# akanimax/thr3ed_atom

Measured on AMD Instinct MI355X. Metric: ray-samples/sec (fwd+bwd) training step, 800x800 images @ 128^3 SH-2 ReLU field, higher is better.
Workload: dtype f32

## Files before the change

### thr3ed_atom_amd/csrc/relu_field_kernels.hip

```cpp
#include <hip/hip_runtime.h>
#include <stdint.h>

#include <atomic>
#include <climits>
#include <cmath>
#include <cstdlib>
#include <type_traits>

#include "relu_field.h"

namespace {

#ifndef RF_FWD_WAVES
#define RF_FWD_WAVES 4
#endif
#ifndef RF_EMIT_WAVES
#define RF_EMIT_WAVES 6
#endif
#ifndef RF_EMIT_G
#define RF_EMIT_G 2
#endif
constexpr int kWave = 64;
constexpr int kWavesPerBlock = 4;
constexpr int kBlock = kWave * kWavesPerBlock;
// ... 2019 lines not shown
}

template <int K, bool ADAM, bool ONE_ROUND, int TH = kBrickThreads, int BX = 8, bool MIRROR = false>
__device__ __forceinline__ void brick_flush(const GridArgs& g, const BrickArgs& a, const float* acc, bool any, int X0, int Y0, int Z0,
                                            float* gdens, float* gfeat) {
  static_assert(!MIRROR || (ADAM && ONE_ROUND && BX == 4), "the mirror write-out rides on the one-round optimizer flush of 4 x 8 x 8 bricks");
  constexpr int C = 3 * K + 1;
  constexpr int CS = (C + 3) / 4 * 4;
  const int B = ONE_ROUND ? 8 : (1 << a.shift);
  const int SY = brick_row_stride(B, C), SX = brick_slab_stride(B, C);
  const int tid = threadIdx.x;
  const bool split = g.layout == RF_LAYOUT_SPLIT;
  if (split && (C & 3) == 0 && (g.dstride & 3) == 0 && (C == 4 || (g.fstride & 3) == 0)) {
    constexpr int QN = C / 4;
    constexpr int QR = QN > 1 ? QN - 1 : 1;
    const int nq = (BX == 4 ? 4 : B) * B * B * QN;
    auto quad_of = [&](int i, int& fx, int& fy, int& fz, int& qd) -> bool {
      const int col = (i >> a.shift) / QN, r = i - col * (B * QN);
      const bool first = r < B;
      fz = first ? r : (r - B) / QR;
      qd = first ? 0 : 1 + (r - B) - fz * QR;
      fx = col >> a.shift;
      fy = col & (B - 1);
      return i < nq && X0 + fx < g.X && Y0 + fy < g.Y && Z0 + fz < g.Z;
    };
    if constexpr (ADAM) {
      constexpr int U = (QN == 7) ? 4 : 1;
      const AdamArgs& ad = a.adam;
      if constexpr (ONE_ROUND) {
        unsigned int bo[QN];
        int lds_at[QN];
        float4 p4[QN];
        vf4 m4[QN], v4[QN];
#pragma unroll
        for (int u = 0; u < QN; ++u) {
          int fx, fy, fz, qd;
          if (u == 0) {
            fx = tid >> 6;
            fy = (tid >> 3) & 7;
            fz = tid & 7;
            qd = 0;
          } else {
            const int j = (u - 1) * TH + tid, col = j / 48, r = j - col * 48;
            fz = r / 6;
            qd = 1 + r - 6 * fz;
            fx = col >> 3;
            fy = col & 7;
          }
          const bool ok = X0 + fx < g.X && Y0 + fy < g.Y && Z0 + fz < g.Z;
          const unsigned int lin = ok ? node_lin(g, X0 + fx, Y0 + fy, Z0 + fz) : 0u;
          const unsigned int o = u == 0 ? __umul24(lin, (unsigned)g.dstride) : __umul24(lin, (unsigned)g.fstride) + 4u * (unsigned)(qd - 1);
          bo[u] = ok ? o * 4u : 0xffffffffu;
          lds_at[u] = fx * SX + fy * SY + fz * CS + 4 * qd;
        }
#pragma unroll
        for (int u = 0; u < QN; ++u) {
          if (bo[u] != 0xffffffffu) {
            const char* pb = reinterpret_cast<const char*>(u == 0 ? ad.p1 : ad.p2);
            const char* mb = reinterpret_cast<const char*>(u == 0 ? ad.m1 : ad.m2);
            const char* vb = reinterpret_cast<const char*>(u == 0 ? ad.v1 : ad.v2);
            p4[u] = *reinterpret_cast<const float4*>(pb + bo[u]);
            m4[u] = __builtin_nontemporal_load(reinterpret_cast<const vf4*>(mb + bo[u]));
            v4[u] = __builtin_nontemporal_load(reinterpret_cast<const vf4*>(vb + bo[u]));
          }
        }
#pragma unroll
        for (int u = 0; u < QN; ++u) {
          if (bo[u] == 0xffffffffu) continue;
          const float4 gq = any ? *reinterpret_cast<const float4*>(&acc[lds_at[u]]) : make_float4(0.f, 0.f, 0.f, 0.f);
          float gg[4] = {gq.x, gq.y, gq.z, gq.w};
          float pn[4] = {p4[u].x, p4[u].y, p4[u].z, p4[u].w};
          if (u == 0 && g.mode == RF_DENSITY_ABS) {
            const float dv = pn[0] * g.rho;
            gg[0] = (dv > 0.f) ? gg[0] : ((dv < 0.f) ? -gg[0] : 0.0f);
          }
          vf4 mn, vn;
#pragma unroll
          for (int c = 0; c < 4; ++c) {
            float mm = m4[u][c], vv = v4[u][c];
            adam_update(pn[c], mm, vv, gg[c], ad.step, ad.b1, ad.b2, ad.eps, ad.inv_bc2_sqrt);
            mn[c] = mm;
            vn[c] = vv;
          }
          char* pb = reinterpret_cast<char*>(u == 0 ? ad.p1 : ad.p2);
          char* mb = reinterpret_cast<char*>(u == 0 ? ad.m1 : ad.m2);
          char* vb = reinterpret_cast<char*>(u == 0 ? ad.v1 : ad.v2);
          *reinterpret_cast<float4*>(pb + bo[u]) = make_float4(pn[0], pn[1], pn[2], pn[3]);
          __builtin_nontemporal_store(mn, reinterpret_cast<vf4*>(mb + bo[u]));
          __builtin_nontemporal_store(vn, reinterpret_cast<vf4*>(vb + bo[u]));
          if constexpr (MIRROR) *reinterpret_cast<float4*>(const_cast<float*>(&acc[lds_at[u]])) = make_float4(pn[0], pn[1], pn[2], pn[3]);
        }
        if constexpr (MIRROR) {
          __syncthreads();
          constexpr int F = 3 * K, FQ = 2 * F, CQ = FQ + 2;
          for (int i = tid; i < 32 * CQ; i += TH) {
            const int col = i / CQ, r = i - col * CQ;
            const int fx = col >> 3, fy = col & 7;
            const float* img = acc + fx * SX + fy * SY;
            const unsigned int lin0 = node_lin(g, X0 + fx, Y0 + fy, Z0);
            float v[4];
            if (r < FQ) {
#pragma unroll
              for (int t = 0; t < 4; ++t) {
                const int e = 4 * r + t;
                const int nz = e / F, f = e - nz * F;
                const int colour = f / K, k = f - colour * K;
                v[t] = img[nz * CS + (k == 0 ? 1 + colour : 4 + colour * (K - 1) + (k - 1))];
              }
              *reinterpret_cast<float4*>(gfeat + (size_t)(__umul24(lin0, (unsigned)F) + 4u * (unsigned)r)) = make_float4(v[0], v[1], v[2], v[3]);
            } else {
              const int z0 = 4 * (r - FQ);
#pragma unroll
              for (int t = 0; t < 4; ++t) v[t] = img[(z0 + t) * CS];
              *reinterpret_cast<float4*>(gdens + (size_t)(lin0 + (unsigned)z0)) = make_float4(v[0], v[1], v[2], v[3]);
            }
          }
        }
        return;
      } else {
      for (int i0 = tid; i0 < nq; i0 += TH * U) {
        unsigned int off[U];
        float4 p4[U];
        vf4 m4[U], v4[U];
#pragma unroll
        for (int u = 0; u < U; ++u) {
          int fx, fy, fz, qd;
          const bool ok = quad_of(i0 + u * TH, fx, fy, fz, qd);
          const unsigned int lin = ok ? node_lin(g, X0 + fx, Y0 + fy, Z0 + fz) : 0u;
          const unsigned int o = qd == 0 ? lin * (unsigned)g.dstride : (lin * (unsigned)g.fstride + 4u * (unsigned)(qd - 1)) | 0x80000000u;
          off[u] = ok ? o : 0xffffffffu;
        }
#pragma unroll
        for (int u = 0; u < U; ++u) {
          if (off[u] != 0xffffffffu) {
            const bool rest = off[u] >> 31;
            const unsigned int o = off[u] & 0x7fffffffu;
#ifdef RF_BRICK_PROFILE
            if (a.stagger & 0x10000) { p4[u] = make_float4(0.f, 0.f, 0.f, 0.f); m4[u] = vf4{0.f, 0.f, 0.f, 0.f}; v4[u] = vf4{1.f, 1.f, 1.f, 1.f}; continue; }
#endif
            p4[u] = *reinterpret_cast<const float4*>((rest ? ad.p2 : ad.p1) + o);
            m4[u] = __builtin_nontemporal_load(reinterpret_cast<const vf4*>((rest ? ad.m2 : ad.m1) + o));
            v4[u] = __builtin_nontemporal_load(reinterpret_cast<const vf4*>((rest ? ad.v2 : ad.v1) + o));
          }
        }
#pragma unroll
        for (int u = 0; u < U; ++u) {
          if (off[u] == 0xffffffffu) continue;
          const bool rest = off[u] >> 31;
          const unsigned int o = off[u] & 0x7fffffffu;
          int fx, fy, fz, qd;
          quad_of(i0 + u * TH, fx, fy, fz, qd);
          const float4 gq = any ? *reinterpret_cast<const float4*>(&acc[fx * SX + fy * SY + fz * CS + 4 * qd]) : make_float4(0.f, 0.f, 0.f, 0.f);
          float gg[4] = {gq.x, gq.y, gq.z, gq.w};
          float pn[4] = {p4[u].x, p4[u].y, p4[u].z, p4[u].w};
          if (!rest && g.mode == RF_DENSITY_ABS) {
            const float dv = pn[0] * g.rho;
            gg[0] = (dv > 0.f) ? gg[0] : ((dv < 0.f) ? -gg[0] : 0.0f);
          }
          vf4 mn, vn;
#ifdef RF_BRICK_PROFILE
          if (a.stagger & 0x40000) {
#pragma unroll
            for (int c = 0; c < 4; ++c) { mn[c] = m4[u][c] + gg[c]; vn[c] = v4[u][c]; pn[c] += gg[c]; }
          } else
#endif
#pragma unroll
          for (int c = 0; c < 4; ++c) {
            float mm = m4[u][c], vv = v4[u][c];
            adam_update(pn[c], mm, vv, gg[c], ad.step, ad.b1, ad.b2, ad.eps, ad.inv_bc2_sqrt);
            mn[c] = mm;
            vn[c] = vv;
          }
#ifdef RF_BRICK_PROFILE
          if (a.stagger & 0x20000) { if (pn[0] == 123.456f) *reinterpret_cast<float4*>((rest ? ad.p2 : ad.p1) + o) = make_float4(mn[0], vn[1], pn[2], pn[3]); continue; }
#endif
          *reinterpret_cast<float4*>((rest ? ad.p2 : ad.p1) + o) = make_float4(pn[0], pn[1], pn[2], pn[3]);
          __builtin_nontemporal_store(mn, reinterpret_cast<vf4*>((rest ? ad.m2 : ad.m1) + o));
          __builtin_nontemporal_store(vn, reinterpret_cast<vf4*>((rest ? ad.v2 : ad.v1) + o));
        }
      }
      }
      return;
    }
    for (int i = tid; i < nq; i += TH) {
      int fx, fy, fz, qd;
      if (!quad_of(i, fx, fy, fz, qd)) continue;
      const long long lin = node_lin(g, X0 + fx, Y0 + fy, Z0 + fz);
      float4 v = any ? *reinterpret_cast<const float4*>(&acc[fx * SX + fy * SY + fz * CS + 4 * qd]) : make_float4(0.f, 0.f, 0.f, 0.f);
      if (qd == 0 && g.mode == RF_DENSITY_ABS) {
        const float dv = g.dens[lin * g.dstride] * g.rho;
        v.x = (dv > 0.f) ? v.x : ((dv < 0.f) ? -v.x : 0.0f);
      }
      const long long off = (qd == 0) ? lin * g.dstride : lin * g.fstride + 4 * (qd - 1);
      if (qd == 0) {
        float4* dst = reinterpret_cast<float4*>(gdens + off);
        if (a.accumulate) {
          const float4 o = *dst;
          v = make_float4(o.x + v.x, o.y + v.y, o.z + v.z, o.w + v.w);
        }
        *dst = v;
      } else {
        float4* dst = reinterpret_cast<float4*>(gfeat + off);
        if (a.accumulate) {
          const float4 o = *dst;
          v = make_float4(o.x + v.x, o.y + v.y, o.z + v.z, o.w + v.w);
        }
        const vf4 v4 = {v.x, v.y, v.z, v.w};
        __builtin_nontemporal_store(v4, reinterpret_cast<vf4*>(dst));
      }
    }
    return;
  }
  const int n_first = split ? 4 : 1;
  const int n_second = C - n_first;
  for (int pass = 0; pass < 2; ++pass) {
    const int nch = pass == 0 ? n_first : n_second;
    if (nch == 0) continue;
    const int run = B * nch;
    float* out = pass == 0 ? gdens : gfeat;
    const long long ostride = pass == 0 ? g.dstride : g.fstride;
    for (int i = tid; i < (BX == 4 ? 4 : B) * B * run; i += TH) {
      const int col = i / run, r = i - col * run;
      const int fz = r / nch, c2 = r - fz * nch;
      const int fx = col >> a.shift, fy = col & (B - 1);
      const int X = X0 + fx, Y = Y0 + fy, Z = Z0 + fz;
      if (X >= g.X || Y >= g.Y || Z >= g.Z) continue;
      int lds_c;
      if (split) {
        lds_c = pass * 4 + c2;
      } else if (pass == 0) {
        lds_c = 0;
      } else {
        const int col3 = c2 / K, kk = c2 - col3 * K;
        lds_c = (kk == 0) ? 1 + col3 : 4 + col3 * (K - 1) + (kk - 1);
      }
      const long long lin = node_lin(g, X, Y, Z);
      float v = any ? acc[fx * SX + fy * SY + fz * CS + lds_c] : 0.0f;
      if (lds_c == 0 && g.mode == RF_DENSITY_ABS) {
        const float dv = g.dens[lin * g.dstride] * g.rho;
        v = (dv > 0.f) ? v : ((dv < 0.f) ? -v : 0.0f);
      }
      float* dst = out + lin * ostride + (long long)c2 * (pass == 1 && !split ? a.fmul : 1);
      *dst = a.accumulate ? (*dst + v) : v;
    }
  }
}

__device__ __forceinline__ uint32_t lds_offset(const void* p) { return (uint32_t)(uintptr_t)p; }
template <int OFF>
__device__ __forceinline__ void lds_request_f32(float& v, uint32_t addr) {
  asm volatile("ds_read_b32 %0, %1 offset:%2" : "+v"(v) : "v"(addr), "n"(OFF));
}
__device__ __forceinline__ void lds_request_u8(uint32_t& v, uint32_t addr) {
  asm volatile("ds_read_u8 %0, %1" : "+v"(v) : "v"(addr));
}
__device__ __forceinline__ void lds_wait(uint32_t& a, uint32_t& b) { asm volatile("s_waitcnt lgkmcnt(0)" : "+v"(a), "+v"(b)); }
__device__ __forceinline__ void lds_wait(float& a, float& b, float& c, float& d, uint32_t& f) {
  asm volatile("s_waitcnt lgkmcnt(0)" : "+v"(a), "+v"(b), "+v"(c), "+v"(d), "+v"(f));
}
__device__ __forceinline__ void lds_wait(float& a, float& b, float& c, float& d, float& e, uint32_t& f) {
  asm volatile("s_waitcnt lgkmcnt(0)" : "+v"(a), "+v"(b), "+v"(c), "+v"(d), "+v"(e), "+v"(f));
}
__device__ __forceinline__ void lds_wait(float& a, float& b, float& c, float& d, float& e, float& e2, float& e3, uint32_t& f) {
  asm volatile("s_waitcnt lgkmcnt(0)" : "+v"(a), "+v"(b), "+v"(c), "+v"(d), "+v"(e), "+v"(e2), "+v"(e3), "+v"(f));
}

constexpr int kGatherBatch = 256;
constexpr int kGatherWtab = 24;
__host__ __device__ constexpr int gather_record_words(int C4) { return C4 + 8; }
typedef float f32x4 __attribute__((ext_vector_type(4)));

__host__ __device__ inline int gather_lds_words(int B, int C, int BX = 8) {
  const int C4 = (C + 3) / 4 * 4;
  const int gb = BX == 4 ? kGatherBatch / 2 : kGatherBatch;
  const int batch = gb * gather_record_words(C4) + (gb + 4) * kGatherWtab;
  const int image = BX == 4 ? 4 * brick_slab_stride(B, C) + 64 : brick_acc_words(B, C);
  return batch > image ? batch : image;
}

template <int K, bool ADAM, bool ONE_ROUND = false, bool SPLIT = false, int BX = 8, bool MIRROR = false>
__global__ __launch_bounds__(BX == 4 ? kBrickThreads / 2 : kBrickThreads, (K > 9 ? 2 : 4)) void brick_gather_kernel(GridArgs g, BrickArgs a, float* gdens, float* gfeat) {
  static_assert(BX == 8 || (BX == 4 && ONE_ROUND && !SPLIT), "4 x 8 x 8 bricks: 8-node y and z edges, one workgroup per brick");
  constexpr int TH = BX == 4 ? kBrickThreads / 2 : kBrickThreads;
  constexpr int NWV = TH / 64;
  constexpr int GB = TH / 2;
  constexpr int GROW = GB + 4;
  constexpr int C = 3 * K + 1;
  constexpr int C4 = (C + 3) / 4 * 4;
  constexpr int QW = record_quads(K);
  constexpr int QN = record_quads(1);
  constexpr int NT = (C4 + 15) / 16;
  static_assert(NT == 1 || NT == 2 || NT == 4, "one, two or four 16-channel blocks (SH degree 0 / base lists, 1-2, 3)");
  constexpr int CS = C4;
  constexpr int NW = GB / 64;
  constexpr bool SEP = BX == 4 && K == 9 && ONE_ROUND && !SPLIT;
  extern __shared__ __attribute__((aligned(16))) float acc[];
  float* rows = acc;
  float* wtab = acc + GB * gather_record_words(C4);
  __shared__ uint32_t s_tmask[GB];
  __shared__ unsigned char s_list[4 * NWV][GB + 24];
  __shared__ __attribute__((aligned(16))) int s_wstart[kMaxRangesKind], s_wcum[kMaxRangesKind + 8];
  __shared__ __attribute__((aligned(16))) int s_nstart[kMaxRangesKind], s_ncum[kMaxRangesKind + 8];
  __shared__ int s_part[4];
  const int B = ONE_ROUND ? 8 : (1 << a.shift);
  const int bshift = ONE_ROUND ? 3 : a.shift;
  const int SY = brick_row_stride(B, C), SX = brick_slab_stride(B, C);

  RF_PROF_START();
  const int tid = threadIdx.x;
  const int lane = tid & (kWave - 1);
  const int wave = tid >> 6;
  const int parts = SPLIT ? a.parts : 1;
  const int part = SPLIT ? (int)(blockIdx.x % (unsigned)parts) : 0;
  const int brick_local = SPLIT ? (int)(blockIdx.x / (unsigned)parts) : (int)blockIdx.x;
  const int brick = a.brick_first + brick_local;
  auto lists_of = [&](int nl) { return SPLIT ? (nl > part ? (nl - part + parts - 1) / parts : 0) : nl; };
  auto list_index = [&](int ll) { return SPLIT ? part + ll * parts : ll; };
  const int nwide_p = lists_of(a.nwide), nnarrow_p = lists_of(a.nnarrow);
  const int bz = brick % a.nbz, by = (brick / a.nbz) % a.nby, bx = brick / (a.nbz * a.nby);
  const int X0 = bx << (BX == 4 ? 2 : bshift), Y0 = by << bshift, Z0 = bz << bshift;
  {
    const int kind = tid >> 7, i = tid & 127;
    int start = 0, cnt = 0;
    if (tid < 256) {
      const int nl = kind ? nnarrow_p : nwide_p;
      if (i < kRangeEntries * nl) {
        const int l = nl == 1 ? 0 : i / kRangeEntries;
        const int li = list_index(l);
        const long long* offs = (!SPLIT && nl == 1) ? (kind ? a.narrow[0].offsets : a.wide[0].offsets) : (kind ? a.narrow[li].offsets : a.wide[li].offsets);
        brick_range_entry(a, offs, bx, by, bz, i - l * kRangeEntries, start, cnt);
      }
    }
    int cum = cnt;
#pragma unroll
    for (int d = 1; d < kWave; d <<= 1) {
      const int up = __shfl_up(cum, d);
      if (lane >= d) cum += up;
    }
    if (wave < 4 && lane == kWave - 1) s_part[wave] = cum;
    __syncthreads();
    if (tid < 256) {
      if (wave & 1) cum += s_part[wave - 1];
      int* st_ = kind ? s_nstart : s_wstart;
      int* cu_ = kind ? s_ncum : s_wcum;
      if (i < kMaxRangesKind) {
        st_[i] = start;
        cu_[i + 1] = cum;
      }
      if (i == 0) cu_[0] = 0;
    }
    __syncthreads();
  }
  const int total = s_wcum[kMaxRangesKind];
  const int total_d = s_ncum[kMaxRangesKind];
  bool any = total > 0 || total_d > 0;
  if (!SPLIT && !any && a.accumulate) return;
  RF_PROF_MARK(0);

  const int npz = B >> 2, npy = B >> 1;
  const int ntiles = BX == 4 ? 16 : (B * B * B) >> 4;
  const int mi = lane & 15;
  const int mdx = mi >> 3, mdy = (mi >> 2) & 1, mdz = mi & 3;
  const int kk = lane >> 4;
  const int jj = lane & 15;

  f32x4 accr[4][NT];
#pragma unroll
  for (int tl = 0; tl < 4; ++tl)
#pragma unroll
    for (int nt = 0; nt < NT; ++nt) accr[tl][nt] = f32x4{0.f, 0.f, 0.f, 0.f};
  f32x4 naccr = f32x4{0.f, 0.f, 0.f, 0.f};

  if (any) {
    const int nba = (total + GB - 1) / GB, nbd = (total_d + GB - 1) / GB;
    uint32_t wprev = 0x00ffffffu;
    const int rec_id = tid & (GB - 1);
    const int half = tid >= GB;

    auto stage = [&](auto expand_tag, auto blocks_tag, float4 q0, float4 q1, float4 q2, int nrec) {
      constexpr bool EXPAND = decltype(expand_tag)::value;
      constexpr bool BLOCKS = decltype(blocks_tag)::value;
      constexpr int RW = gather_record_words(EXPAND ? C4 : 4);
      if (half == 0) {
        uint32_t tm = 0, wnow = 0x00ffffffu;
        float* wcol = wtab + rec_id;
#pragma unroll
        for (int ax = 0; ax < 3; ++ax) {
          const int c1 = (int)((wprev >> (8 * ax)) & 0xffu);
          if (c1 != 0xff) {
            if (c1 >= 1) wcol[(ax * 8 + c1 - 1) * GROW] = 0.0f;
            if (c1 < (BX == 4 && ax == 0 ? 4 : B)) wcol[(ax * 8 + c1) * GROW] = 0.0f;
          }
        }
        if (rec_id < nrec) {
          const float idx[3] = {q0.x, q0.y, q0.z};
          const int org[3] = {X0, Y0, Z0};
          uint32_t pb[3];
          wnow = 0;
#pragma unroll
          for (int ax = 0; ax < 3; ++ax) {
            const float fl = floorf(idx[ax]);
            const int c = (int)fl - org[ax];
            const int sh = (BLOCKS && ax > 0) || ax == 2 ? 2 : 1;
            uint32_t bits = 0;
            if (c >= 0) {
              wcol[(ax * 8 + c) * GROW] = (fl + 1.0f) - idx[ax];
              bits |= 1u << (c >> sh);
            }
            if (c + 1 < (BX == 4 && ax == 0 ? 4 : B)) {
              wcol[(ax * 8 + c + 1) * GROW] = idx[ax] - fl;
              bits |= 1u << ((c + 1) >> sh);
            }
            pb[ax] = bits;
            wnow |= (uint32_t)(c + 1) << (8 * ax);
          }
          if constexpr (BLOCKS) {
            if (pb[0]) tm = ((pb[1] & 1u) ? pb[2] : 0u) | ((pb[1] & 2u) ? pb[2] << 2 : 0u);
          } else {
            uint32_t yz = 0;
#pragma unroll
            for (int py = 0; py < 4; ++py)
              if ((pb[1] >> py) & 1u) yz |= pb[2] << (py * npz);
#pragma unroll
            for (int px = 0; px < 4; ++px)
              if ((pb[0] >> px) & 1u) tm |= yz << (px * npy * npz);
          }
        }
        wprev = wnow;
        s_tmask[rec_id] = tm;
      }
      float* row = rows + rec_id * RW;
      if constexpr (EXPAND) {
        const float graw[3] = {q1.x, q1.y, q1.z};
        constexpr int NQ = C4 / 4;
        if (half == 0) {
          *reinterpret_cast<float4*>(row) = make_float4(q0.w, graw[0] * kC0, graw[1] * kC0, graw[2] * kC0);
        } else {
          float Y[16];
          sh_basis<K>(q1.w, q2.x, q2.y, Y);
#pragma unroll
          for (int q = 1; q < NQ; ++q) {
            float v[4];
#pragma unroll
            for (int x = 0; x < 4; ++x) v[x] = (4 * q + x < C) ? record_channel<K>(4 * q + x, q0.w, graw, Y) : 0.0f;
            *reinterpret_cast<float4*>(row + 4 * q) = make_float4(v[0], v[1], v[2], v[3]);
          }
        }
      } else {
        if (half == 0) *reinterpret_cast<float4*>(row) = q1;
      }
    };
    auto process = [&](auto wide_tag, int nrec) {
      constexpr bool WIDE = decltype(wide_tag)::value;
      constexpr int RW = gather_record_words(WIDE ? C4 : 4);
      constexpr int NTW = WIDE ? NT : 1;
      RF_PROF_MARK(7);
      __syncthreads();
      RF_PROF_MARK(2);
      int cnt[4] = {0, 0, 0, 0};
#if defined(RF_BRICK_PROFILE) || defined(RF_BRICK_ABLATE)
      const bool no_lists = a.stagger & 0x200000, no_tiles = a.stagger & 0x100000;
#else
      constexpr bool no_lists = false, no_tiles = false;
#endif
      if (!no_lists)
#pragma unroll
      for (int wd = 0; wd < NW; ++wd) {
        if (wd * 64 >= nrec) break;
        const uint32_t tmv = s_tmask[wd * 64 + lane] >> wave;
#pragma unroll
        for (int tl = 0; tl < 4; ++tl) {
          const bool hit = (tmv >> (NWV * tl)) & 1u;
          const unsigned long long m = __ballot(hit);
          const int pos = cnt[tl] + __builtin_amdgcn_mbcnt_hi((uint32_t)(m >> 32), __builtin_amdgcn_mbcnt_lo((uint32_t)m, 0));
          if (hit) s_list[(tl * NWV + wave)][pos] = (unsigned char)(wd * 64 + lane);
          cnt[tl] += __popcll(m);
        }
      }
#pragma unroll
      for (int tl = 0; tl < 4; ++tl)
        if (lane < 8) s_list[(tl * NWV + wave)][cnt[tl] + lane] = 0;
#pragma unroll
      for (int tl = 0; tl < 4; ++tl) {
        const int t = (tl * NWV + wave);
        const int n = cnt[tl];
        if (t < ntiles && n > 0 && !no_tiles) {
          const int pz = t % npz, py = (t / npz) % npy, px = t / (npz * npy);
          const float* wx = wtab + (2 * px + mdx) * GROW;
          const float* wy = wtab + (8 + 2 * py + mdy) * GROW;
          const float* wz = wtab + (16 + 4 * pz + mdz) * GROW;
          const float* gbase = rows + (WIDE ? jj : (jj & 3));
          const uint32_t a_list = lds_offset(s_list[t]) + kk;
          const uint32_t a_x = lds_offset(wx), a_y = lds_offset(wy), a_z = lds_offset(wz), a_g = lds_offset(gbase);
          const int nq = (n + 3) >> 2;
          uint32_t ra = 0, rb = 0;
          float aw0 = 0.f, aw1 = 0.f, aw2 = 0.f, bw0 = 0.f, bw1 = 0.f, bw2 = 0.f;
          float ag0 = 0.f, ag1 = 0.f, ag2 = 0.f, ag3 = 0.f, bg0 = 0.f, bg1 = 0.f, bg2 = 0.f, bg3 = 0.f;
          auto request_ops = [&](float& w0, float& w1, float& w2, float& g0, float& g1, float& g2, float& g3, uint32_t r) {
            lds_request_f32<0>(w0, a_x + 4 * r);
            lds_request_f32<0>(w1, a_y + 4 * r);
            lds_request_f32<0>(w2, a_z + 4 * r);
            const uint32_t a_row = a_g + (uint32_t)__umul24(r, RW * 4);
            lds_request_f32<0>(g0, a_row);
            if constexpr (NTW > 1) lds_request_f32<64>(g1, a_row);
            if constexpr (NTW > 2) {
              lds_request_f32<128>(g2, a_row);
              lds_request_f32<192>(g3, a_row);
            }
          };
          auto wait_ops = [&](float& w0, float& w1, float& w2, float& g0, float& g1, float& g2, float& g3, uint32_t& r) {
            if constexpr (NTW > 2)
              lds_wait(w0, w1, w2, g0, g1, g2, g3, r);
            else
              lds_wait(w0, w1, w2, g0, g1, r);
          };
          auto multiply = [&](float w0, float w1, float w2, float g0, float g1, float g2, float g3, int q) {
            const float wv = (w0 * w1) * w2;
            const float wa = (4 * q + kk < n) ? wv : 0.0f;
            const float ga = (WIDE || jj < 4) ? g0 : 0.0f;
            accr[tl][0] = __builtin_amdgcn_mfma_f32_16x16x4f32(wa, ga, accr[tl][0], 0, 0, 0);
            if constexpr (NTW > 1) accr[tl][1] = __builtin_amdgcn_mfma_f32_16x16x4f32(wa, g1, accr[tl][1], 0, 0, 0);
            if constexpr (NTW > 2) {
              accr[tl][2] = __builtin_amdgcn_mfma_f32_16x16x4f32(wa, g2, accr[tl][2], 0, 0, 0);
              accr[tl][3] = __builtin_amdgcn_mfma_f32_16x16x4f32(wa, g3, accr[tl][3], 0, 0, 0);
            }
          };
          lds_request_u8(ra, a_list);
          lds_request_u8(rb, a_list + 4);
          lds_wait(ra, rb);
          request_ops(aw0, aw1, aw2, ag0, ag1, ag2, ag3, ra);
          for (int q = 0; q < nq; q += 2) {
            wait_ops(aw0, aw1, aw2, ag0, ag1, ag2, ag3, rb);
            lds_request_u8(ra, a_list + 4 * q + 8);
            request_ops(bw0, bw1, bw2, bg0, bg1, bg2, bg3, rb);
            multiply(aw0, aw1, aw2, ag0, ag1, ag2, ag3, q);
            if (q + 1 < nq) {
              wait_ops(bw0, bw1, bw2, bg0, bg1, bg2, bg3, ra);
              lds_request_u8(rb, a_list + 4 * q + 12);
              request_ops(aw0, aw1, aw2, ag0, ag1, ag2, ag3, ra);
              multiply(bw0, bw1, bw2, bg0, bg1, bg2, bg3, q + 1);
            }
          }
          wait_ops(aw0, aw1, aw2, ag0, ag1, ag2, ag3, ra);
          wait_ops(bw0, bw1, bw2, bg0, bg1, bg2, bg3, rb);
        }
      }
      RF_PROF_MARK(3);
      __syncthreads();
      RF_PROF_MARK(2);
    };
    auto process_blocks = [&](int nrec) {
      constexpr int RW = gather_record_words(4);
      RF_PROF_MARK(7);
      __syncthreads();
      RF_PROF_MARK(2);
#if defined(RF_BRICK_PROFILE) || defined(RF_BRICK_ABLATE)
      const bool no_lists = a.stagger & 0x200000, no_tiles = a.stagger & 0x100000;
#else
      constexpr bool no_lists = false, no_tiles = false;
#endif
      unsigned char* list = s_list[wave];
      int n = 0;
      if (!no_lists)
#pragma unroll
        for (int wd = 0; wd < NW; ++wd) {
          if (wd * 64 >= nrec) break;
          const bool hit = (s_tmask[wd * 64 + lane] >> wave) & 1u;
          const unsigned long long m = __ballot(hit);
          const int pos = n + __builtin_amdgcn_mbcnt_hi((uint32_t)(m >> 32), __builtin_amdgcn_mbcnt_lo((uint32_t)m, 0));
          if (hit) list[pos] = (unsigned char)(wd * 64 + lane);
          n += __popcll(m);
        }
      if (lane < 8) list[n + lane] = 0;
      if (n > 0 && !no_tiles) {
        const uint32_t a_list = lds_offset(list) + kk;
        const uint32_t a_x = lds_offset(wtab + (mi & 3) * GROW);
        const uint32_t a_y = lds_offset(wtab + (8 + 4 * (wave >> 1) + (jj >> 2)) * GROW);
        const uint32_t a_z = lds_offset(wtab + (16 + 4 * (wave & 1) + (jj & 3)) * GROW);
        const uint32_t a_g = lds_offset(rows + (mi >> 2));
        const int nq = (n + 3) >> 2;
        uint32_t ra = 0, rb = 0;
        float xa = 0.f, ya = 0.f, za = 0.f, ga = 0.f, xb = 0.f, yb = 0.f, zb = 0.f, gb = 0.f;
        auto request_ops = [&](float& wx, float& wy, float& wz, float& g, uint32_t r) {
          lds_request_f32<0>(wx, a_x + 4 * r);
          lds_request_f32<0>(wy, a_y + 4 * r);
          lds_request_f32<0>(wz, a_z + 4 * r);
          lds_request_f32<0>(g, a_g + (uint32_t)__umul24(r, RW * 4));
        };
        auto multiply = [&](float wx, float wy, float wz, float g, int q) {
          const float av = g * wx;
          const float aa = (4 * q + kk < n) ? av : 0.0f;
          naccr = __builtin_amdgcn_mfma_f32_16x16x4f32(aa, wy * wz, naccr, 0, 0, 0);
        };
        lds_request_u8(ra, a_list);
        lds_request_u8(rb, a_list + 4);
        lds_wait(ra, rb);
        request_ops(xa, ya, za, ga, ra);
        for (int q = 0; q < nq; q += 2) {
          lds_wait(xa, ya, za, ga, rb);
          lds_request_u8(ra, a_list + 4 * q + 8);
          request_ops(xb, yb, zb, gb, rb);
          multiply(xa, ya, za, ga, q);
          if (q + 1 < nq) {
            lds_wait(xb, yb, zb, gb, ra);
            lds_request_u8(rb, a_list + 4 * q + 12);
            request_ops(xa, ya, za, ga, ra);
            multiply(xb, yb, zb, gb, q + 1);
          }
        }
        lds_wait(xa, ya, za, ga, ra);
        lds_wait(xb, yb, zb, gb, rb);
      }
      RF_PROF_MARK(3);
      __syncthreads();
      RF_PROF_MARK(2);
    };
    using Yes = std::integral_constant<bool, true>;
    using No = std::integral_constant<bool, false>;

    int sri = 0, dri = 0;
    int rlo = 0, rhi = 0, dlo = 0, dhi = 0;
    const float4* rptr = a.wide[SPLIT ? min(part, kMaxListsPerKind - 1) : 0].rec;
    const float4* dptr = a.narrow[SPLIT ? min(part, kMaxListsPerKind - 1) : 0].rec;
    float4 w0 = make_float4(0.f, 0.f, 0.f, 0.f), w1 = w0, w2 = w0, d0 = w0, d1 = w0;
    auto range_of = [&](const int* cum, int v, int nlists, int from) -> int {
      if (nlists == 1) {
        const int4* c4 = reinterpret_cast<const int4*>(cum);
        const int4 c0 = c4[0], c1 = c4[1], c2 = c4[2], c3 = c4[3];
        return (c0.y <= v) + (c0.z <= v) + (c0.w <= v) + (c1.x <= v) + (c1.y <= v) + (c1.z <= v) + (c1.w <= v) + (c2.x <= v) + (c2.y <= v) + (c2.z <= v) +
               (c2.w <= v) + (c3.x <= v) + (c3.y <= v) + (c3.z <= v);
      }
      int i = from;
      while (cum[i] > v) --i;
      while (cum[i + 1] <= v) ++i;
      return i;
    };
    auto fetch_wide = [&](int s) {
      const int nrec = min(GB, total - s * GB);
      const int v = s * GB + min(rec_id, nrec - 1);
      if (v < rlo || v >= rhi) {
        sri = range_of(s_wcum, v, nwide_p, sri);
        rlo = s_wcum[sri];
        rhi = s_wcum[sri + 1];
        rptr = ((!SPLIT && a.nwide == 1) ? a.wide[0].rec : a.wide[list_index(sri / kRangeEntries)].rec) + (long long)(s_wstart[sri] - rlo) * QW;
      }
      const float4* p = rptr + (long long)v * QW;
      w0 = load_f4<RF_NT_RECORD_LOAD>(p);
      w1 = load_f4<RF_NT_RECORD_LOAD>(p + 1);
      if constexpr (QW > 2) w2 = load_f4<RF_NT_RECORD_LOAD>(p + 2);
    };
    auto fetch_narrow = [&](int sd) {
      const int nrec = min(GB, total_d - sd * GB);
      const int v = sd * GB + min(rec_id, nrec - 1);
      if (v < dlo || v >= dhi) {
        dri = range_of(s_ncum, v, nnarrow_p, dri);
        dlo = s_ncum[dri];
        dhi = s_ncum[dri + 1];
        dptr = ((!SPLIT && a.nnarrow == 1) ? a.narrow[0].rec : a.narrow[list_index(dri / kRangeEntries)].rec) + (long long)(s_nstart[dri] - dlo) * QN;
      }
      const float4* p = dptr + (long long)v * QN;
      d0 = load_f4<RF_NT_RECORD_LOAD>(p);
      d1 = load_f4<RF_NT_RECORD_LOAD>(p + 1);
    };
    if (nbd > 0) fetch_narrow(0);
    if (nba > 0) fetch_wide(0);
    for (int i = tid; i < GROW * kGatherWtab / 4; i += TH) reinterpret_cast<float4*>(wtab)[i] = make_float4(0.f, 0.f, 0.f, 0.f);
    __syncthreads();
    for (int s = 0; s < nba; ++s) {
      const int nrec = min(GB, total - s * GB);
      if constexpr (K > 1)
        stage(Yes{}, No{}, w0, w1, w2, nrec);
      else
        stage(No{}, No{}, w0, w1, w2, nrec);
      RF_PROF_MARK(1);
      fetch_wide(min(s + 1, nba - 1));
      RF_PROF_MARK(6);
      process(Yes{}, nrec);
    }
    for (int sd = 0; sd < nbd; ++sd) {
      const int nrec = min(GB, total_d - sd * GB);
      stage(No{}, std::integral_constant<bool, SEP>{}, d0, d1, d1, nrec);
      RF_PROF_MARK(1);
      fetch_narrow(min(sd + 1, nbd - 1));
      RF_PROF_MARK(6);
      if constexpr (SEP)
        process_blocks(nrec);
      else
        process(No{}, nrec);
    }
#pragma unroll
    for (int tl = 0; tl < 4; ++tl) {
      const int t = (tl * NWV + wave);
      if (t < ntiles) {
        const int pz = t % npz, py = (t / npz) % npy, px = t / (npz * npy);
#pragma unroll
        for (int nt = 0; nt < NT; ++nt) {
          const int ch = 16 * nt + jj;
#pragma unroll
          for (int e = 0; e < 4; ++e) {
            const int i = 4 * kk + e;
            const int nx = 2 * px + (i >> 3), ny = 2 * py + ((i >> 2) & 1), nz = 4 * pz + (i & 3);
            if (ch < CS) acc[nx * SX + ny * SY + nz * CS + ch] = accr[tl][nt][e];
          }
        }
      }
    }
    if constexpr (SEP) {
      if (total_d > 0) {
        __syncthreads();
        const int ny = 4 * (wave >> 1) + (jj >> 2), nz = 4 * (wave & 1) + (jj & 3);
#pragma unroll
        for (int e = 0; e < 4; ++e) acc[e * SX + ny * SY + nz * CS + kk] += naccr[e];
      }
    }
    __syncthreads();
    RF_PROF_MARK(5);
  }
  if constexpr (SPLIT) {
    const int words = brick_acc_words(B, C);
    int* state = a.part_state + (long long)brick_local * (1 + parts);
    unsigned long long* images = reinterpret_cast<unsigned long long*>(a.partial + (long long)brick_local * parts * words);
    const int pairs = words / 2;
    __shared__ int s_arrival;
    if (any) {
      unsigned long long* mine = images + (long long)part * pairs;
      const unsigned long long* src = reinterpret_cast<const unsigned long long*>(acc);
      for (int i = tid; i < pairs; i += TH) __hip_atomic_store(mine + i, src[i], __ATOMIC_RELAXED, __HIP_MEMORY_SCOPE_AGENT);
      if (tid == 0) __hip_atomic_store(&state[1 + part], 1, __ATOMIC_RELAXED, __HIP_MEMORY_SCOPE_AGENT);
    }
    asm volatile("s_waitcnt vmcnt(0)" ::: "memory");
    __syncthreads();
    if (tid == 0) s_arrival = __hip_atomic_fetch_add(&state[0], 1, __ATOMIC_RELAXED, __HIP_MEMORY_SCOPE_AGENT);
    __syncthreads();
    if (s_arrival != parts - 1) return;
    for (int j = 0; j < parts; ++j) {
      if (j == part) continue;
      if (__hip_atomic_load(&state[1 + j], __ATOMIC_RELAXED, __HIP_MEMORY_SCOPE_AGENT) == 0) continue;
      const unsigned long long* other = images + (long long)j * pairs;
      float2* own = reinterpret_cast<float2*>(acc);
      for (int i = tid; i < pairs; i += TH) {
        const unsigned long long o = __hip_atomic_load(other + i, __ATOMIC_RELAXED, __HIP_MEMORY_SCOPE_AGENT);
        float2 v = any ? own[i] : make_float2(0.f, 0.f);
        v.x += __uint_as_float((uint32_t)o);
        v.y += __uint_as_float((uint32_t)(o >> 32));
        own[i] = v;
      }
      any = true;
      __syncthreads();
    }
    if (tid <= parts) state[tid] = 0;
    __syncthreads();
  }
#if defined(RF_BRICK_PROFILE) || defined(RF_BRICK_ABLATE)
  if (!(a.stagger & 0x400000))
#endif
  brick_flush<K, ADAM, ONE_ROUND, TH, BX, MIRROR>(g, a, acc, any, X0, Y0, Z0, gdens, gfeat);
  RF_PROF_MARK(4);
  RF_PROF_END();
}

__device__ __forceinline__ long long channel_offset(const GridArgs& g, unsigned int lin, int ch, int K, bool& in_first) {
  if (g.layout == RF_LAYOUT_REFERENCE) {
    in_first = ch == 0;
    if (ch == 0) return (long long)lin * g.dstride;
    if (ch < 4) return (long long)lin * g.fstride + (long long)(ch - 1) * K;
    const int j = ch - 4, colour = j / (K - 1), kk = 1 + j - colour * (K - 1);
    return (long long)lin * g.fstride + (long long)colour * K + kk;
  }
  in_first = ch < 4;
  return ch < 4 ? (long long)lin * g.dstride + ch : (long long)lin * g.fstride + (ch - 4);
}

struct UpsampleAxis {
  int i0, i1;
  float w0, w1;
};
__device__ __forceinline__ UpsampleAxis upsample_axis(int dst, int in_size, float scale) {
  float src = fmaf(scale, (float)dst + 0.5f, -0.5f);
  src = src < 0.0f ? 0.0f : src;
  UpsampleAxis a;
  a.i0 = min((int)floorf(src), in_size - 1);
  a.i1 = a.i0 + (a.i0 < in_size - 1 ? 1 : 0);
  const float lambda = fminf(fmaxf(src - (float)a.i0, 0.0f), 1.0f);
  a.w0 = 1.0f - lambda;
  a.w1 = lambda;
  return a;
}

__global__ void upsample_grid_kernel(GridArgs src, GridArgs dst, float* dst_first, float* dst_second, long long total) {
  const int C = dst.F + 1, K = dst.F / 3;
  const float sx = (float)src.X / (float)dst.X, sy = (float)src.Y / (float)dst.Y, sz = (float)src.Z / (float)dst.Z;
  for (long long it = (long long)blockIdx.x * blockDim.x + threadIdx.x; it < total; it += (long long)gridDim.x * blockDim.x) {
    const int ch = (int)(it % C);
    long long node = it / C;
    const int z = (int)(node % dst.Z);
    node /= dst.Z;
    const int y = (int)(node % dst.Y), x = (int)(node / dst.Y);
    const UpsampleAxis ax = upsample_axis(x, src.X, sx), ay = upsample_axis(y, src.Y, sy), az = upsample_axis(z, src.Z, sz);
    auto at = [&](int xi, int yi, int zi) -> float {
      bool first;
      const long long off = channel_offset(src, node_lin(src, xi, yi, zi), ch, K, first);
      return (first ? src.dens : src.feat)[off];
    };
    float val[8], wgt[8];
#pragma unroll
    for (int k = 0; k < 8; ++k) {
      const int dx = k >> 2, dy = (k >> 1) & 1, dz = k & 1;
      val[k] = at(dx ? ax.i1 : ax.i0, dy ? ay.i1 : ay.i0, dz ? az.i1 : az.i0);
      wgt[k] = ((dx ? ax.w1 : ax.w0) * (dy ? ay.w1 : ay.w0)) * (dz ? az.w1 : az.w0);
    }
    int uc;
    if (ch == 0) {
      uc = dst.F;
    } else if (ch < 4) {
      uc = (ch - 1) * K;
    } else {
      const int j = ch - 4, colour = j / (K - 1);
      uc = colour * K + 1 + (j - colour * (K - 1));
    }
    float v;
    if (uc < (C & ~7)) {
      v = fmaf(val[7], wgt[7], val[6] * wgt[6]);
#pragma unroll
      for (int k = 5; k >= 0; --k) v = fmaf(val[k], wgt[k], v);
    } else {
      v = fmaf(val[0], wgt[0], val[1] * wgt[1]);
#pragma unroll
      for (int k = 2; k < 8; ++k) v = fmaf(val[k], wgt[k], v);
    }
    bool first;
    const long long off = channel_offset(dst, node_lin(dst, x, y, z), ch, K, first);
    (first ? dst_first : dst_second)[off] = v;
  }
}

__global__ void convert_grid_kernel(GridArgs src, GridArgs dst, float* dst_first, float* dst_second, unsigned int nodes) {
  const int C = dst.F + 1, K = dst.F / 3;
  const int ch = threadIdx.x;
  const bool linear = !src.bricked && !dst.bricked;
  for (unsigned int node = blockIdx.x * blockDim.y + threadIdx.y; node < nodes; node += gridDim.x * blockDim.y) {
    if (ch >= C) continue;
    unsigned int ls = node, ld = node;
    if (!linear) {
      const unsigned int z = node % (unsigned)dst.Z, t = node / (unsigned)dst.Z;
      const unsigned int y = t % (unsigned)dst.Y, x = t / (unsigned)dst.Y;
      ls = node_lin(src, (int)x, (int)y, (int)z);
      ld = node_lin(dst, (int)x, (int)y, (int)z);
    }
    bool sf, df;
    const long long so = channel_offset(src, ls, ch, K, sf);
    const long long doff = channel_offset(dst, ld, ch, K, df);
    (df ? dst_first : dst_second)[doff] = (sf ? src.dens : src.feat)[so];
  }
}

template <int K>
__global__ void reference_to_split_kernel(const float* __restrict__ dens, const float* __restrict__ feat, long long dstride, long long fstride,
                                          float4* __restrict__ base, float4* __restrict__ rest, unsigned int nodes) {
  constexpr int QN = (3 * K + 1) / 4;
  constexpr int KR = K > 1 ? K - 1 : 1;
  const unsigned int total = nodes * QN;
  for (unsigned int it = blockIdx.x * blockDim.x + threadIdx.x; it < total; it += gridDim.x * blockDim.x) {
    const unsigned int node = it / QN, q = it - node * QN;
    const float* f = feat + (long long)node * fstride;
    if (q == 0) {
      base[node] = make_float4(dens[(long long)node * dstride], f[0], f[K], f[2 * K]);
    } else {
      float v[4];
#pragma unroll
      for (int x = 0; x < 4; ++x) {
        const unsigned int r = 4 * (q - 1) + x;
        const unsigned int colour = r / KR, k = r - colour * KR + 1;
        v[x] = f[colour * K + k];
      }
      rest[(long long)node * (QN - 1) + (q - 1)] = make_float4(v[0], v[1], v[2], v[3]);
    }
  }
}

template <int K>
__global__ void split_to_reference_kernel(const float4* __restrict__ base, const float4* __restrict__ rest, float* __restrict__ dens,
                                          float* __restrict__ feat, long long dstride, long long fstride, unsigned int nodes) {
  constexpr int QN = (3 * K + 1) / 4;
  constexpr int KR = K > 1 ? K - 1 : 1;
  const unsigned int total = nodes * QN;
  for (unsigned int it = blockIdx.x * blockDim.x + threadIdx.x; it < total; it += gridDim.x * blockDim.x) {
    const unsigned int node = it / QN, q = it - node * QN;
    float* f = feat + (long long)node * fstride;
    if (q == 0) {
      const float4 v = base[node];
      dens[(long long)node * dstride] = v.x;
      f[0] = v.y;
      f[K] = v.z;
      f[2 * K] = v.w;
    } else {
      const float4 v4 = rest[(long long)node * (QN - 1) + (q - 1)];
      const float v[4] = {v4.x, v4.y, v4.z, v4.w};
#pragma unroll
      for (int x = 0; x < 4; ++x) {
        const unsigned int r = 4 * (q - 1) + x;
        const unsigned int colour = r / KR, k = r - colour * KR + 1;
        f[colour * K + k] = v[x];
      }
    }
  }
}

template <int K>
__global__ void split_to_reference_quads_kernel(const float* __restrict__ base, const float* __restrict__ rest, float4* __restrict__ dens4,
                                                float4* __restrict__ feat4, unsigned int nodes) {
  constexpr unsigned int F = 3 * K, R = F - 3;
  constexpr unsigned int KR = K > 1 ? K - 1 : 1;
  const unsigned int fq = nodes * F / 4, dq = nodes / 4;
  for (unsigned int it = blockIdx.x * blockDim.x + threadIdx.x; it < fq + dq; it += gridDim.x * blockDim.x) {
    float v[4];
    if (it < fq) {
#pragma unroll
      for (unsigned int x = 0; x < 4; ++x) {
        const unsigned int f = 4 * it + x, node = f / F, c = f - node * F;
        const unsigned int colour = c / K, k = c - colour * K;
        v[x] = (k == 0) ? base[node * 4 + 1 + colour] : rest[node * R + colour * KR + (k - 1)];
      }
      feat4[it] = make_float4(v[0], v[1], v[2], v[3]);
    } else {
      const unsigned int n0 = 4 * (it - fq);
      dens4[it - fq] = make_float4(base[n0 * 4], base[n0 * 4 + 4], base[n0 * 4 + 8], base[n0 * 4 + 12]);
    }
  }
}

struct QueryCorner {
  long long lin;
  float w;
  bool ok;
};

__device__ __forceinline__ void query_cell(const float p[3], const GridArgs& g, int i0[3], float w0[3], float w1[3]) {
  const int dims[3] = {g.X, g.Y, g.Z};
#pragma unroll
  for (int a = 0; a < 3; ++a) {
    const float q = p[a] * g.nscale[a] + g.nbias[a];
    const float idx = ((q + 1.0f) * (float)dims[a] - 1.0f) / 2.0f;
    const float fl = floorf(idx);
    w1[a] = idx - fl;
    w0[a] = (fl + 1.0f) - idx;
    i0[a] = (int)fminf(fmaxf(fl, -2.0f), (float)dims[a]);
  }
}

__device__ __forceinline__ QueryCorner query_corner(int k, const int i0[3], const float w0[3], const float w1[3],
                                                    const GridArgs& g) {
  const int dx = k & 1, dy = (k >> 1) & 1, dz = k >> 2;
  const int ix = i0[0] + dx, iy = i0[1] + dy, iz = i0[2] + dz;
  QueryCorner c;
  c.ok = ix >= 0 && ix < g.X && iy >= 0 && iy < g.Y && iz >= 0 && iz < g.Z;
  c.lin = node_lin(g, min(max(ix, 0), g.X - 1), min(max(iy, 0), g.Y - 1), min(max(iz, 0), g.Z - 1));
  c.w = ((dx ? w1[0] : w0[0]) * (dy ? w1[1] : w0[1])) * (dz ? w1[2] : w0[2]);
  return c;
}

__device__ __forceinline__ long long query_offset(int c, long long lin, const GridArgs& g, bool* in_first) {
  const int F = g.F, K = F / 3;
  if (c == F) {
    *in_first = true;
    return lin * g.dstride;
  }
  if (g.layout == RF_LAYOUT_SPLIT) {
    const int ch = c / K, k = c % K;
    if (k == 0) {
      *in_first = true;
      return lin * g.dstride + 1 + ch;
    }
    *in_first = false;
    return lin * g.fstride + ch * (K - 1) + (k - 1);
  }
  *in_first = false;
  return lin * g.fstride + c;
}

__device__ __forceinline__ float density_post(float pre, int mode) {
  if (mode == RF_DENSITY_RELU) return fmaxf(pre, 0.0f);
  if (mode == RF_DENSITY_SOFTPLUS) return (pre > 20.0f) ? pre : log1pf(expf(pre));
  return pre;
}
// ... 2679 lines not shown
```

Baseline: 16.30 billion.

## Stage narrow base-channel batches with all threads in separable brick path

In the separable (BX==4, SH-2, one-round) gather path, narrow base-channel records are now staged one per thread (TH records per batch instead of GB), using a dedicated weight table, byte masks and lists aliased into the existing shared buffers. This halves the number of narrow batches and their barriers, and lets all threads stage instead of only half. The risks are added shared-memory aliasing complexity and byte-sized indices, which a static_assert guards, plus an extra table clear before the narrow pass.

```diff
diff --git a/thr3ed_atom_amd/csrc/relu_field_kernels.hip b/thr3ed_atom_amd/csrc/relu_field_kernels.hip
--- a/thr3ed_atom_amd/csrc/relu_field_kernels.hip
+++ b/thr3ed_atom_amd/csrc/relu_field_kernels.hip
@@ -2345,6 +2345,15 @@
   __shared__ __attribute__((aligned(16))) int s_wstart[kMaxRangesKind], s_wcum[kMaxRangesKind + 8];
   __shared__ __attribute__((aligned(16))) int s_nstart[kMaxRangesKind], s_ncum[kMaxRangesKind + 8];
   __shared__ int s_part[4];
+  constexpr int GBN = SEP ? TH : GB;
+  constexpr int BROW = TH + 4;
+  constexpr int NWB = TH / 64;
+  float* btab = acc;
+  float* brows = acc + 20 * BROW;
+  unsigned char* bmask = reinterpret_cast<unsigned char*>(s_tmask);
+  unsigned char(*blist)[TH + 24] = reinterpret_cast<unsigned char(*)[TH + 24]>(&s_list[0][0]);
+  static_assert(!SEP || (20 * BROW + 4 * TH <= GB * gather_record_words(C4) + GROW * kGatherWtab && TH <= kGatherBatch && NWV * (TH + 24) <= 4 * NWV * (GB + 24)),
+                "the base-channel batch of the separable form fits the full-width batch's buffers, its indices a byte");
   const int B = ONE_ROUND ? 8 : (1 << a.shift);
   const int bshift = ONE_ROUND ? 3 : a.shift;
   const int SY = brick_row_stride(B, C), SX = brick_slab_stride(B, C);
@@ -2415,14 +2424,13 @@
   f32x4 naccr = f32x4{0.f, 0.f, 0.f, 0.f};
 
   if (any) {
-    const int nba = (total + GB - 1) / GB, nbd = (total_d + GB - 1) / GB;
+    const int nba = (total + GB - 1) / GB, nbd = (total_d + GBN - 1) / GBN;
     uint32_t wprev = 0x00ffffffu;
     const int rec_id = tid & (GB - 1);
     const int half = tid >= GB;
 
-    auto stage = [&](auto expand_tag, auto blocks_tag, float4 q0, float4 q1, float4 q2, int nrec) {
+    auto stage = [&](auto expand_tag, float4 q0, float4 q1, float4 q2, int nrec) {
       constexpr bool EXPAND = decltype(expand_tag)::value;
-      constexpr bool BLOCKS = decltype(blocks_tag)::value;
       constexpr int RW = gather_record_words(EXPAND ? C4 : 4);
       if (half == 0) {
         uint32_t tm = 0, wnow = 0x00ffffffu;
@@ -2444,7 +2452,7 @@
           for (int ax = 0; ax < 3; ++ax) {
             const float fl = floorf(idx[ax]);
             const int c = (int)fl - org[ax];
-            const int sh = (BLOCKS && ax > 0) || ax == 2 ? 2 : 1;
+            const int sh = ax == 2 ? 2 : 1;
             uint32_t bits = 0;
             if (c >= 0) {
               wcol[(ax * 8 + c) * GROW] = (fl + 1.0f) - idx[ax];
@@ -2457,17 +2465,13 @@
             pb[ax] = bits;
             wnow |= (uint32_t)(c + 1) << (8 * ax);
           }
-          if constexpr (BLOCKS) {
-            if (pb[0]) tm = ((pb[1] & 1u) ? pb[2] : 0u) | ((pb[1] & 2u) ? pb[2] << 2 : 0u);
-          } else {
-            uint32_t yz = 0;
-#pragma unroll
-            for (int py = 0; py < 4; ++py)
-              if ((pb[1] >> py) & 1u) yz |= pb[2] << (py * npz);
-#pragma unroll
-            for (int px = 0; px < 4; ++px)
-              if ((pb[0] >> px) & 1u) tm |= yz << (px * npy * npz);
-          }
+          uint32_t yz = 0;
+#pragma unroll
+          for (int py = 0; py < 4; ++py)
+            if ((pb[1] >> py) & 1u) yz |= pb[2] << (py * npz);
+#pragma unroll
+          for (int px = 0; px < 4; ++px)
+            if ((pb[0] >> px) & 1u) tm |= yz << (px * npy * npz);
         }
         wprev = wnow;
         s_tmask[rec_id] = tm;
@@ -2492,6 +2496,45 @@
       } else {
         if (half == 0) *reinterpret_cast<float4*>(row) = q1;
       }
+    };
+    auto stage_blocks = [&](float4 q0, float4 q1, int nrec) {
+      uint32_t tm = 0, wnow = 0x00ffffffu;
+      float* wcol = btab + tid;
+      constexpr int first_row[3] = {0, 4, 12}, nodes[3] = {4, 8, 8};
+#pragma unroll
+      for (int ax = 0; ax < 3; ++ax) {
+        const int c1 = (int)((wprev >> (8 * ax)) & 0xffu);
+        if (c1 != 0xff) {
+          if (c1 >= 1) wcol[(first_row[ax] + c1 - 1) * BROW] = 0.0f;
+          if (c1 < nodes[ax]) wcol[(first_row[ax] + c1) * BROW] = 0.0f;
+        }
+      }
+      if (tid < nrec) {
+        const float idx[3] = {q0.x, q0.y, q0.z};
+        const int org[3] = {X0, Y0, Z0};
+        uint32_t pb[3];
+        wnow = 0;
+#pragma unroll
+        for (int ax = 0; ax < 3; ++ax) {
+          const float fl = floorf(idx[ax]);
+          const int c = (int)fl - org[ax];
+          uint32_t bits = 0;
+          if (c >= 0) {
+            wcol[(first_row[ax] + c) * BROW] = (fl + 1.0f) - idx[ax];
+            bits |= 1u << (c >> 2);
+          }
+          if (c + 1 < nodes[ax]) {
+            wcol[(first_row[ax] + c + 1) * BROW] = idx[ax] - fl;
+            bits |= 1u << ((c + 1) >> 2);
+          }
+          pb[ax] = bits;
+          wnow |= (uint32_t)(c + 1) << (8 * ax);
+        }
+        if (pb[0]) tm = ((pb[1] & 1u) ? pb[2] : 0u) | ((pb[1] & 2u) ? pb[2] << 2 : 0u);
+      }
+      wprev = wnow;
+      bmask[tid] = (unsigned char)tm;
+      *reinterpret_cast<float4*>(brows + 4 * tid) = q1;
     };
     auto process = [&](auto wide_tag, int nrec) {
       constexpr bool WIDE = decltype(wide_tag)::value;
@@ -2593,7 +2636,6 @@
       RF_PROF_MARK(2);
     };
     auto process_blocks = [&](int nrec) {
-      constexpr int RW = gather_record_words(4);
       RF_PROF_MARK(7);
       __syncthreads();
       RF_PROF_MARK(2);
@@ -2602,13 +2644,13 @@
 #else
       constexpr bool no_lists = false, no_tiles = false;
 #endif
-      unsigned char* list = s_list[wave];
+      unsigned char* list = blist[wave];
       int n = 0;
       if (!no_lists)
 #pragma unroll
-        for (int wd = 0; wd < NW; ++wd) {
+        for (int wd = 0; wd < NWB; ++wd) {
           if (wd * 64 >= nrec) break;
-          const bool hit = (s_tmask[wd * 64 + lane] >> wave) & 1u;
+          const bool hit = (bmask[wd * 64 + lane] >> wave) & 1u;
           const unsigned long long m = __ballot(hit);
           const int pos = n + __builtin_amdgcn_mbcnt_hi((uint32_t)(m >> 32), __builtin_amdgcn_mbcnt_lo((uint32_t)m, 0));
           if (hit) list[pos] = (unsigned char)(wd * 64 + lane);
@@ -2617,10 +2659,10 @@
       if (lane < 8) list[n + lane] = 0;
       if (n > 0 && !no_tiles) {
         const uint32_t a_list = lds_offset(list) + kk;
-        const uint32_t a_x = lds_offset(wtab + (mi & 3) * GROW);
-        const uint32_t a_y = lds_offset(wtab + (8 + 4 * (wave >> 1) + (jj >> 2)) * GROW);
-        const uint32_t a_z = lds_offset(wtab + (16 + 4 * (wave & 1) + (jj & 3)) * GROW);
-        const uint32_t a_g = lds_offset(rows + (mi >> 2));
+        const uint32_t a_x = lds_offset(btab + (mi & 3) * BROW);
+        const uint32_t a_y = lds_offset(btab + (4 + 4 * (wave >> 1) + (jj >> 2)) * BROW);
+        const uint32_t a_z = lds_offset(btab + (12 + 4 * (wave & 1) + (jj & 3)) * BROW);
+        const uint32_t a_g = lds_offset(brows + (mi >> 2));
         const int nq = (n + 3) >> 2;
         uint32_t ra = 0, rb = 0;
         float xa = 0.f, ya = 0.f, za = 0.f, ga = 0.f, xb = 0.f, yb = 0.f, zb = 0.f, gb = 0.f;
@@ -2628,7 +2670,7 @@
           lds_request_f32<0>(wx, a_x + 4 * r);
           lds_request_f32<0>(wy, a_y + 4 * r);
           lds_request_f32<0>(wz, a_z + 4 * r);
-          lds_request_f32<0>(g, a_g + (uint32_t)__umul24(r, RW * 4));
+          lds_request_f32<0>(g, a_g + 16 * r);
         };
         auto multiply = [&](float wx, float wy, float wz, float g, int q) {
           const float av = g * wx;
@@ -2693,8 +2735,8 @@
       if constexpr (QW > 2) w2 = load_f4<RF_NT_RECORD_LOAD>(p + 2);
     };
     auto fetch_narrow = [&](int sd) {
-      const int nrec = min(GB, total_d - sd * GB);
-      const int v = sd * GB + min(rec_id, nrec - 1);
+      const int nrec = min(GBN, total_d - sd * GBN);
+      const int v = sd * GBN + min(SEP ? tid : rec_id, nrec - 1);
       if (v < dlo || v >= dhi) {
         dri = range_of(s_ncum, v, nnarrow_p, dri);
         dlo = s_ncum[dri];
@@ -2707,22 +2749,34 @@
     };
     if (nbd > 0) fetch_narrow(0);
     if (nba > 0) fetch_wide(0);
-    for (int i = tid; i < GROW * kGatherWtab / 4; i += TH) reinterpret_cast<float4*>(wtab)[i] = make_float4(0.f, 0.f, 0.f, 0.f);
-    __syncthreads();
+    if (!SEP || nba > 0) {
+      for (int i = tid; i < GROW * kGatherWtab / 4; i += TH) reinterpret_cast<float4*>(wtab)[i] = make_float4(0.f, 0.f, 0.f, 0.f);
+      __syncthreads();
+    }
     for (int s = 0; s < nba; ++s) {
       const int nrec = min(GB, total - s * GB);
       if constexpr (K > 1)
-        stage(Yes{}, No{}, w0, w1, w2, nrec);
+        stage(Yes{}, w0, w1, w2, nrec);
       else
-        stage(No{}, No{}, w0, w1, w2, nrec);
+        stage(No{}, w0, w1, w2, nrec);
       RF_PROF_MARK(1);
       fetch_wide(min(s + 1, nba - 1));
       RF_PROF_MARK(6);
       process(Yes{}, nrec);
     }
+    if constexpr (SEP) {
+      if (nbd > 0) {
+#pragma unroll
+        for (int r = 0; r < 20; ++r) btab[r * BROW + tid] = 0.0f;
+        wprev = 0x00ffffffu;
+      }
+    }
     for (int sd = 0; sd < nbd; ++sd) {
-      const int nrec = min(GB, total_d - sd * GB);
-      stage(No{}, std::integral_constant<bool, SEP>{}, d0, d1, d1, nrec);
+      const int nrec = min(GBN, total_d - sd * GBN);
+      if constexpr (SEP)
+        stage_blocks(d0, d1, nrec);
+      else
+        stage(No{}, d0, d1, d1, nrec);
       RF_PROF_MARK(1);
       fetch_narrow(min(sd + 1, nbd - 1));
       RF_PROF_MARK(6);
```

Measured after the change: 16.47 billion (median of 6 runs). +1.1%, better.
